# jzhou316/meta-gcn

Hardware: AMD Instinct MI355X
Metric: edges/sec GCN fwd+bwd, 10M-edge synth graph F=128, at 1/2/4/8 MI355X (higher is better)
Workload: dtype f32; 1 GPU; config2: Erdos-Renyi N=1M, E=10M (+1M self-loops), F=128, 3-layer GCN (sm, add, bias, ReLU) fwd+bwd; nodes=1000000, edges=10000000, nnz=11000000, feat=128, layers=3, global_batch=1, parallelism=single

## Files before the change

meta-gcn_amd/csrc/fused.hip:

```cpp

#include <string>

#include "mgcn_internal.h"
#include "x6.h"

#ifndef MGCN_NT_AUX
#define MGCN_NT_AUX 2
#endif
#ifndef MGCN_NT_OUT
#define MGCN_NT_OUT 2
#endif

namespace mgcn {
namespace {

using namespace x6;

constexpr int kXwF = 128;
constexpr int kXwRows = 32;
constexpr int kXwWaves = 8;
constexpr int kXwThreads = 64 * kXwWaves;
constexpr int kXwImg = kXwRows * 256;
constexpr int kXwStageLd = kXwF + 8;
constexpr int kXwStage = kXwRows * kXwStageLd * 4;
// ... 312 lines not shown
        wb[u] = bcast_g(mwb, grp, k & 31);
        const uint32_t oa = k < na ? (uint32_t)ca * ldx_b + 16u * gl : 0xfffffff0u;
        const uint32_t ob = k < nb ? (uint32_t)cb * ldx_b + 16u * gl : 0xfffffff0u;
        xa[u] = __builtin_bit_cast(float4, __builtin_amdgcn_raw_buffer_load_b128(rx, oa, 0, 0));
        xb[u] = __builtin_bit_cast(float4, __builtin_amdgcn_raw_buffer_load_b128(rx, ob, 0, 0));
        if constexpr (MAXM) {
          const int sa = bcast_g(msa, grp, k & 31);
          const int sb = bcast_g(msb, grp, k & 31);
          ba[u] = win[k < na ? (int64_t)sa * 4 + (gl >> 3) : 0];
          bb[u] = win[k < nb ? (int64_t)sb * 4 + (gl >> 3) : 0];
        }
      }
#pragma unroll
      for (int u = 0; u < U; ++u) {
        if constexpr (MAXM) {
          const uint32_t qa = ba[u] >> (4 * (gl & 7)), qb = bb[u] >> (4 * (gl & 7));
          xa[u].x = (qa & 1u) ? xa[u].x : 0.0f;
          xa[u].y = (qa & 2u) ? xa[u].y : 0.0f;
          xa[u].z = (qa & 4u) ? xa[u].z : 0.0f;
          xa[u].w = (qa & 8u) ? xa[u].w : 0.0f;
          xb[u].x = (qb & 1u) ? xb[u].x : 0.0f;
          xb[u].y = (qb & 2u) ? xb[u].y : 0.0f;
          xb[u].z = (qb & 4u) ? xb[u].z : 0.0f;
          xb[u].w = (qb & 8u) ? xb[u].w : 0.0f;
        }
        if (k0 + u < na) {
          aa[0] = __fadd_rn(aa[0], __fmul_rn(xa[u].x, wa[u]));
          aa[1] = __fadd_rn(aa[1], __fmul_rn(xa[u].y, wa[u]));
          aa[2] = __fadd_rn(aa[2], __fmul_rn(xa[u].z, wa[u]));
          aa[3] = __fadd_rn(aa[3], __fmul_rn(xa[u].w, wa[u]));
        }
        if (k0 + u < nb) {
          ab[0] = __fadd_rn(ab[0], __fmul_rn(xb[u].x, wb[u]));
          ab[1] = __fadd_rn(ab[1], __fmul_rn(xb[u].y, wb[u]));
          ab[2] = __fadd_rn(ab[2], __fmul_rn(xb[u].z, wb[u]));
          ab[3] = __fadd_rn(ab[3], __fmul_rn(xb[u].w, wb[u]));
        }
      }
    }
  }
}

struct RowSeq {
  int64_t base;
  int64_t step;
  int64_t n_rows;
  __device__ __forceinline__ int64_t row(int64_t k) const { return base + (k >> 1) * step + 16 * (k & 1); }
};

__device__ __forceinline__ int64_t my_chunks(int64_t n_chunks) {
  return blockIdx.x < n_chunks ? (n_chunks - 1 - blockIdx.x) / gridDim.x + 1 : 0;
}

__device__ __forceinline__ void store_row_terms(char *img_base, int lr, int gl, const float (&v)[4]) {
  uint32_t hi[2], mid[2], lo[2];
  split3_pair(f32x2{v[0], v[1]}, hi[0], mid[0], lo[0]);
  split3_pair(f32x2{v[2], v[3]}, hi[1], mid[1], lo[1]);
  char *img = img_base + img_off(lr, gl >> 1) + 8 * (gl & 1);
  *reinterpret_cast<uint2 *>(img) = make_uint2(hi[0], hi[1]);
  *reinterpret_cast<uint2 *>(img + kXwImg) = make_uint2(mid[0], mid[1]);
  *reinterpret_cast<uint2 *>(img + 2 * kXwImg) = make_uint2(lo[0], lo[1]);
}

__device__ __forceinline__ void mfma_rows(const char *img, const bf16x8 (&b)[3], int ks, int l16,
                                          int g4, f32x4_t (&acc)[2]) {
#pragma unroll
  for (int t = 0; t < 2; ++t) {
    const int off = img_off(16 * t + l16, 4 * ks + g4);
    const bf16x8 ah = *reinterpret_cast<const bf16x8 *>(img + off);
    const bf16x8 am = *reinterpret_cast<const bf16x8 *>(img + kXwImg + off);
    const bf16x8 al = *reinterpret_cast<const bf16x8 *>(img + 2 * kXwImg + off);
    acc[t] = mfma16_x6(ah, am, al, b[0], b[1], b[2], acc[t]);
  }
}

constexpr int kXfBuf = 3 * kXwImg;
constexpr int kXfStageOff = 2 * kXfBuf;
constexpr int kXfLds = kXfStageOff + 2 * kXfStage;
static_assert(2 * kXfLds <= 160 * 1024, "two forward workgroups per CU");

struct XwArgs {
  int64_t n_rows;
  const int64_t *rowptr;
  const int32_t *col;
  const float *w;
  const float *X;
  int64_t ldx;
  int64_t n_cols;
  const float *W;
  int64_t ldw;
  const float *bias;
  float *Y;
  int64_t ldy;
  uint32_t *relu_mask;
  float *Z;
  int64_t ldz;
  int mean;
  int relu;
  const uint32_t *pk;
  uint32_t pk_bytes, pk_rbits, pk_head;
  uint32_t pk_base[64];
};

template <int U, bool PK = false>
__global__ __launch_bounds__(kXwThreads, 2 * kXwPerCU) void spmm_xw_fwd_kernel(const XwArgs a) {
  __shared__ __attribute__((aligned(16))) char lds[kXfLds];
  const int tid = threadIdx.x;
  const int lane = tid & 63;
  const int wave = __builtin_amdgcn_readfirstlane(tid >> 6);
  const int gl = lane & 31, grp = lane >> 5;
  const int l16 = lane & 15, g4 = lane >> 4;
  const int64_t n_chunks = (a.n_rows + kXwRows - 1) / kXwRows;
  const bool has_b = a.bias != nullptr;
  const auto rx = buf_rsrc(PK ? nullptr : a.X, PK ? 0u : (uint32_t)(a.n_cols * a.ldx * 4));
  const uint32_t ldx_b = (uint32_t)a.ldx * 4u;
  Pk128 pk{};
  u32x2 hh[PK ? U : 1];
  if constexpr (PK) {
    pk.r = buf_rsrc(a.pk, a.pk_bytes);
    pk.rbits = a.pk_rbits;
    pk.head = a.pk_head;
    pk.base = a.pk_base[lane];
  }

  const int ncol = 16 * wave + l16;
  bf16x8 wb[4][3];
  {
    const float *wp = a.W + (int64_t)(8 * g4) * a.ldw + ncol;
#pragma unroll
    for (int ks = 0; ks < 4; ++ks) {
      float v[8];
#pragma unroll
      for (int j = 0; j < 8; ++j) v[j] = wp[(int64_t)(32 * ks + j) * a.ldw];
      split3_bf16(v, wb[ks][0], wb[ks][1], wb[ks][2]);
    }
  }
  const float bcol = has_b ? a.bias[ncol] : 0.0f;

  auto flush = [&](int64_t c, const float *stage) {
    const int64_t r0 = c * kXwRows;
    const int64_t left = a.n_rows - r0;
    const uint32_t rows_in = (uint32_t)(left >= kXwRows ? kXwRows : left);
    const auto ry = buf_rsrc(a.Y + r0 * a.ldy, rows_in * (uint32_t)a.ldy * 4u);
#pragma unroll
    for (int m = 0; m < 2; ++m) {
      const int lr = 16 * m + (tid >> 5);
      const float4 v = *reinterpret_cast<const float4 *>(stage + lr * kXwF + 4 * gl);
      __builtin_amdgcn_raw_buffer_store_b128(__builtin_bit_cast(u32x4, v), ry,
                                             4 * (int)(lr * a.ldy + 4 * gl), 0, MGCN_NT_OUT);
      if (a.relu_mask != nullptr) {
        const uint32_t m0 = (uint32_t)(__ballot(v.x > 0.0f) >> (32 * grp));
        const uint32_t m1 = (uint32_t)(__ballot(v.y > 0.0f) >> (32 * grp));
        const uint32_t m2 = (uint32_t)(__ballot(v.z > 0.0f) >> (32 * grp));
        const uint32_t m3 = (uint32_t)(__ballot(v.w > 0.0f) >> (32 * grp));
        if (gl == 0 && (uint32_t)lr < rows_in)
          *reinterpret_cast<uint4 *>(a.relu_mask + (r0 + lr) * 4) = make_uint4(m0, m1, m2, m3);
      }
    }
  };

  const int64_t n_my = my_chunks(n_chunks);
  const RowSeq seq{(int64_t)blockIdx.x * kXwRows + 2 * wave + grp, (int64_t)gridDim.x * kXwRows,
                   a.n_rows};
  RowMeta cur, nxt;
  meta_rowptr(a.rowptr, seq.row(0), seq.row(0) < a.n_rows, cur);
  if constexpr (PK) {
    meta_first_pk(pk, a.col, a.w, gl, cur);
    pk128_headers<U>(pk, cur.mc, grp, 0, cur.deg < 32 ? cur.deg : 32, 8u * (uint32_t)(gl >> 3), hh);
  } else {
    meta_first(a.col, a.w, gl, cur);
  }
  meta_rowptr(a.rowptr, seq.row(1), seq.row(1) < a.n_rows, nxt);
  int it = 0;
  for (int64_t chunk = blockIdx.x; chunk < n_chunks; chunk += gridDim.x, ++it) {
    char *buf = lds + (it & 1) * kXfBuf;
    float *stage = reinterpret_cast<float *>(lds + kXfStageOff + (it & 1) * kXfStage);

#pragma unroll 1
    for (int p = 0; p < 2; ++p) {
      const int lr = 16 * p + 2 * wave + grp;
      const int64_t k = 2 * it + p;
      if constexpr (PK)
        meta_first_pk(pk, a.col, a.w, gl, nxt);
      else
        meta_first(a.col, a.w, gl, nxt);
      RowMeta nn;
      const int64_t r2 = seq.row(k + 2);
      meta_rowptr(a.rowptr, r2, r2 < a.n_rows && k + 2 < 2 * n_my, nn);
      float acc[4];
      if constexpr (PK)
        gather_row_meta_pk<U>(pk, a.col, a.w, cur, nxt, gl, grp, acc, hh);
      else
        gather_row_meta<U>(rx, ldx_b, a.col, a.w, cur, gl, grp, acc);
      if (a.Z != nullptr) {
        const int64_t r0 = chunk * kXwRows;
        const int64_t left = a.n_rows - r0;
        const uint32_t rows_in = (uint32_t)(left >= kXwRows ? kXwRows : left);
        const auto rz = buf_rsrc(a.Z + r0 * a.ldz, rows_in * (uint32_t)a.ldz * 4u);
        __builtin_amdgcn_raw_buffer_store_b128(
            __builtin_bit_cast(u32x4, make_float4(acc[0], acc[1], acc[2], acc[3])), rz,
            4 * (int)(lr * a.ldz + 4 * gl), 0, MGCN_NT_AUX);
      }
      if (a.mean) {
        const float c = (float)(cur.deg > 1 ? cur.deg : 1);
#pragma unroll
        for (int j = 0; j < 4; ++j) acc[j] = __fdiv_rn(acc[j], c);
      }
      store_row_terms(buf, lr, gl, acc);
      cur = nxt;
      nxt = nn;
    }
    __syncthreads();
    if (it > 0)
      flush(chunk - gridDim.x, reinterpret_cast<const float *>(lds + kXfStageOff +
                                                                ((it + 1) & 1) * kXfStage));

    f32x4_t acc2[2];
#pragma unroll
    for (int t = 0; t < 2; ++t)
#pragma unroll
      for (int r = 0; r < 4; ++r) acc2[t][r] = 0.0f;
#pragma unroll
    for (int ks = 0; ks < 4; ++ks) mfma_rows(buf, wb[ks], ks, l16, g4, acc2);
#pragma unroll
    for (int t = 0; t < 2; ++t)
#pragma unroll
      for (int r = 0; r < 4; ++r) {
        float v = acc2[t][r];
        if (has_b) v = __fadd_rn(v, bcol);
        if (a.relu) v = (v < 0.0f) ? 0.0f : v;
        stage[(16 * t + 4 * g4 + r) * kXwF + ncol] = v;
      }
  }
  if (it > 0) {
    __syncthreads();
    flush(blockIdx.x + (int64_t)(it - 1) * gridDim.x,
          reinterpret_cast<const float *>(lds + kXfStageOff + ((it + 1) & 1) * kXfStage));
  }
}

constexpr int kXbHOff = 3 * kXwImg;
constexpr int kXbMaskOff = 6 * kXwImg;
constexpr int kXbDivOff = kXbMaskOff + kXwRows * 16;
constexpr int kXbStageOff = kXbDivOff + kXwRows * 4;
constexpr int kXbColsumOff = kXbStageOff + kXwStage;
constexpr int kXbLds = kXbColsumOff + kXwThreads * 16;
static_assert(2 * kXbLds <= 160 * 1024, "two backward workgroups per CU");

struct XbArgs {
  int64_t n_rows;
  const int64_t *rowptr;
  const int32_t *col;
  const float *w;
  const float *row_scale;
  const float *dY;
  int64_t lddy;
  int64_t n_cols;
  const float *X;
  int64_t ldx;
  const float *W;
  int64_t ldw;
  float *dX;
  int64_t lddx;
  const uint32_t *relu_mask;
  const float *row_div;
  float *dw_partial;
  float *colsum_partial;
  const uint32_t *win_mask;
  const int32_t *slot_map;
  const uint32_t *pk;
  uint32_t pk_bytes, pk_rbits, pk_head;
  uint32_t pk_base[64];
};

#ifdef MGCN_XW_PROFILE
__device__ unsigned long long g_xprof[2][64][6];
#define XPROF(it, k)                                                                      \
  if (blockIdx.x == 0 && (wave == 0 || wave == 7) && (it) < 64 && lane == 0)              \
    g_xprof[wave == 7][it][k] = __builtin_readcyclecounter();
#else
#define XPROF(it, k)
#endif

template <int U, bool DX, int EPI, bool MAXM, bool DW = true, bool PK = false>
__global__ __launch_bounds__(kXwThreads, 2 * kXwPerCU) void spmm_xw_bwd_kernel(const XbArgs a) {
  static_assert(!PK || (!DW && !MAXM), "the packed gather serves the dX-only adjoint");
  __shared__ __attribute__((aligned(16))) char lds[kXbLds];
  const int tid = threadIdx.x;
  const int lane = tid & 63;
  const int wave = __builtin_amdgcn_readfirstlane(tid >> 6);
  const int gl = lane & 31, grp = lane >> 5;
// ... 224 lines not shown
            stage[lc * kXwStageLd + kXwF + 4] = *reinterpret_cast<const float *>(lds + kXbDivOff + 4 * lc);
        }
      }
    }
    XPROF(it, 4);
    __syncthreads();
    XPROF(it, 5);
  }
  if constexpr (DX) {
    if (it > 0) flush(blockIdx.x + (int64_t)(it - 1) * gridDim.x);
  }

  float *slab = a.dw_partial + (int64_t)blockIdx.x * kXwF * kXwF;
#pragma unroll
  for (int s = 0; s < (DW ? 2 : 0); ++s)
#pragma unroll
    for (int r = 0; r < 16; ++r) {
      const int row = 32 * ti + (r & 3) + 8 * (r >> 2) + 4 * h;
      slab[row * kXwF + 32 * (tj0 + s) + lc] = accw[s][r];
    }
  if constexpr (DX && EPI != EPI_STORE) {
    __syncthreads();
    const float *red = reinterpret_cast<const float *>(lds + kXbColsumOff);
    if (tid < kXwF) {
      float c = 0.0f;
#pragma unroll
      for (int q = 0; q < 16; ++q) c = __fadd_rn(c, red[4 * (32 * q + (tid >> 2)) + (tid & 3)]);
      a.colsum_partial[(int64_t)blockIdx.x * kXwF + tid] = c;
    }
  }
}

int g_xw_unroll = 5;
int g_xw_pk_unroll = 3;
int g_xw_pk_bwd_unroll = 3;

int xw_grid() {
  int dev = 0, cus = 256;
  if (hipGetDevice(&dev) != hipSuccess ||
      hipDeviceGetAttribute(&cus, hipDeviceAttributeMultiprocessorCount, dev) != hipSuccess)
    cus = 256;
  return kXwPerCU * cus;
}

template <int U, bool PK = false>
int launch_xw(const XwArgs &a, hipStream_t s) {
  const int64_t n_chunks = (a.n_rows + kXwRows - 1) / kXwRows;
  int64_t grid = xw_grid();
  if (grid > n_chunks) grid = n_chunks;
  hipLaunchKernelGGL((spmm_xw_fwd_kernel<U, PK>), dim3((unsigned)grid), dim3(kXwThreads), 0, s, a);
  return check_launch("spmm_xw_fwd_kernel");
}

template <int U, bool DX, int EPI, bool MAXM, bool DW = true, bool PK = false>
int launch_xb(const XbArgs &a, int grid, hipStream_t s) {
  hipLaunchKernelGGL((spmm_xw_bwd_kernel<U, DX, EPI, MAXM, DW, PK>), dim3((unsigned)grid),
                     dim3(kXwThreads), 0, s, a);
  return check_launch("spmm_xw_bwd_kernel");
}

template <int U, bool PK = false>
int launch_xb_dx(const XbArgs &a, int epi, int grid, hipStream_t s) {
  if (epi == EPI_RELU_DIV) return launch_xb<U, true, EPI_RELU_DIV, false, false, PK>(a, grid, s);
  if (epi == EPI_RELU) return launch_xb<U, true, EPI_RELU, false, false, PK>(a, grid, s);
  return launch_xb<U, true, EPI_STORE, false, false, PK>(a, grid, s);
}

template <int U, bool MAXM>
int launch_xb_m(const XbArgs &a, int epi, int grid, hipStream_t s) {
  if (a.dX == nullptr) return launch_xb<U, false, EPI_STORE, MAXM>(a, grid, s);
  if (epi == EPI_RELU_DIV) return launch_xb<U, true, EPI_RELU_DIV, MAXM>(a, grid, s);
  if (epi == EPI_RELU) return launch_xb<U, true, EPI_RELU, MAXM>(a, grid, s);
  return launch_xb<U, true, EPI_STORE, MAXM>(a, grid, s);
}

template <int U>
int launch_xb_u(const XbArgs &a, int epi, int grid, hipStream_t s) {
  return a.win_mask != nullptr ? launch_xb_m<U, true>(a, epi, grid, s)
                               : launch_xb_m<U, false>(a, epi, grid, s);
}

constexpr int kBsDws = 2, kBsDwsH = 3, kBsDwsM = 4;
#ifndef MGCN_DS_MASK_RING
#define MGCN_DS_MASK_RING 1
#endif
constexpr int kBsImgSet = 3 * kXwImg;
constexpr int kDsXLd = kXwF + 4;
constexpr int kDsXOff = kBsImgSet;
constexpr int kDsMaskOff = kDsXOff + kXwRows * kDsXLd * 4;
constexpr int kDsDivOff = kDsMaskOff + kXwRows * 16;
constexpr int kDsRingBuf = kDsDivOff + kXwRows * 4;
constexpr int kDsWOff = 2 * kDsRingBuf;
constexpr int kDsCtrOff = kDsWOff + kXwF * kDsXLd * 4;
constexpr int kDsLds = kDsCtrOff + 64;
static_assert(kDsLds <= 160 * 1024, "one DWS workgroup per CU");
static_assert(16 * kXwF * 4 <= kDsWOff, "column-sum fold fits in the ring");
constexpr int kBsNG = 8, kBsNM = 8;
constexpr int kBsThreads = 64 * (kBsNG + kBsNM);

__device__ __forceinline__ int bs_lds_load(const int *p) {
  return __builtin_amdgcn_readfirstlane(
      __hip_atomic_load(p, __ATOMIC_RELAXED, __HIP_MEMORY_SCOPE_WORKGROUP));
}

__device__ __forceinline__ bool bs_wait_ge(const int *p, int target, int *abort_word,
                                           uint32_t limit) {
// ... 13 lines not shown
__device__ __forceinline__ int bs_signal(int *p, int v, int lane) {
  asm volatile("s_waitcnt lgkmcnt(0)" ::: "memory");
  int old = 0;
  if (lane == 0) old = __hip_atomic_fetch_add(p, v, __ATOMIC_RELAXED, __HIP_MEMORY_SCOPE_WORKGROUP);
  return __builtin_amdgcn_readfirstlane(old);
}

__device__ __forceinline__ f32x4_t mfma16_x6_at(const bf16x8 (&w)[3], const bf16x8 &xh,
                                               const bf16x8 &xm, const bf16x8 &xl, f32x4_t c) {
  c = __builtin_amdgcn_mfma_f32_16x16x32_bf16(w[0], xl, c, 0, 0, 0);
  c = __builtin_amdgcn_mfma_f32_16x16x32_bf16(w[2], xh, c, 0, 0, 0);
  c = __builtin_amdgcn_mfma_f32_16x16x32_bf16(w[1], xm, c, 0, 0, 0);
  c = __builtin_amdgcn_mfma_f32_16x16x32_bf16(w[0], xm, c, 0, 0, 0);
  c = __builtin_amdgcn_mfma_f32_16x16x32_bf16(w[1], xh, c, 0, 0, 0);
  return __builtin_amdgcn_mfma_f32_16x16x32_bf16(w[0], xh, c, 0, 0, 0);
}

struct XbsArgs {
  XbArgs b;
  float *hcs_partial;
  int dbg;
  uint32_t spin;
  unsigned *err;
};

template <int U, int EPI, int MODE>
__global__ __launch_bounds__(kBsThreads) void spmm_xw_bwd_ws_kernel(const XbsArgs A) {
  constexpr bool HCS = MODE == kBsDwsH;
  constexpr bool MAXM = MODE == kBsDwsM;
  constexpr bool MRING = MGCN_DS_MASK_RING;
  constexpr int kRing = kDsRingBuf;
  constexpr int kDbgMask = MAXM ? ~0 : mgcn::kDbgMask;
  const XbArgs &a = A.b;
  __shared__ __attribute__((aligned(16))) char lds[kDsLds];
  const int tid = threadIdx.x;
  const int lane = tid & 63;
  const int wave = __builtin_amdgcn_readfirstlane(tid >> 6);
  const int gl = lane & 31, grp = lane >> 5;
  const int l16 = lane & 15, g4 = lane >> 4;
  int *ctr = reinterpret_cast<int *>(lds + kDsCtrOff);
  int *filled = ctr, *mdone = ctr + 2, *freed = ctr + 4, *abort_word = ctr + 8;
  if (tid < 16) ctr[tid] = 0;
#pragma unroll
  for (int j = 0; j < 4; ++j) {
    const int e = tid + kBsThreads * j;
    const float4 v = *reinterpret_cast<const float4 *>(a.W + (int64_t)(e >> 5) * a.ldw + 4 * (e & 31));
    *reinterpret_cast<float4 *>(lds + kDsWOff + 4 * ((e >> 5) * kDsXLd + 4 * (e & 31))) = v;
  }
  __syncthreads();

  const int64_t n_chunks = (a.n_rows + kXwRows - 1) / kXwRows;
  const int64_t n_my = my_chunks(n_chunks);
  auto chunk_of = [&](int64_t i) { return (int64_t)blockIdx.x + i * gridDim.x; };
  auto rows_in = [&](int64_t c) -> uint32_t {
    const int64_t r = a.n_rows - c * kXwRows;
    return (uint32_t)(r <= 0 ? 0 : r >= kXwRows ? kXwRows : r);
  };

  float cs[4] = {0.0f, 0.0f, 0.0f, 0.0f};
  float hc[4] = {0.0f, 0.0f, 0.0f, 0.0f};
  f32x16 accw[2];
#pragma unroll
  for (int s = 0; s < 2; ++s)
#pragma unroll
    for (int r = 0; r < 16; ++r) accw[s][r] = 0.0f;

  if (wave < kBsNG) {
    const int64_t n_quads = 8 * n_my;
    auto row_of = [&](int64_t k, int second) -> int64_t {
      const int64_t q = wave + kBsNG * k;
      return chunk_of(q >> 3) * kXwRows + 4 * (q & 7) + 2 * second + grp;
    };
    const auto rdy = buf_rsrc(a.dY, (uint32_t)(a.n_cols * a.lddy * 4));
    const uint32_t ldy_b = (uint32_t)a.lddy * 4u;
    RowMeta cur[2] = {}, nxt[2] = {};
#pragma unroll
    for (int j = 0; j < 2; ++j) {
      meta_rowptr(a.rowptr, row_of(0, j), row_of(0, j) < a.n_rows && wave < n_quads, cur[j]);
      if constexpr (MAXM)
        meta_first_m(a.col, a.w, a.slot_map, gl, cur[j]);
      else
        meta_first(a.col, a.w, gl, cur[j]);
      meta_rowptr(a.rowptr, row_of(1, j), row_of(1, j) < a.n_rows && wave + kBsNG < n_quads,
                  nxt[j]);
    }
    int64_t k = 0;
    for (int64_t q = wave; q < n_quads; q += kBsNG, ++k) {
      RowMeta nn[2];
#pragma unroll
      for (int j = 0; j < 2; ++j) {
        if constexpr (MAXM)
          meta_first_m(a.col, a.w, a.slot_map, gl, nxt[j]);
        else
          meta_first(a.col, a.w, gl, nxt[j]);
        const int64_t r2 = row_of(k + 2, j);
        meta_rowptr(a.rowptr, r2, r2 < a.n_rows && q + 2 * kBsNG < n_quads, nn[j]);
      }
      const int64_t i = q >> 3;
      const int64_t c = chunk_of(i);
      const int64_t r0 = c * kXwRows;
      const int lr0 = 4 * (int)(q & 7) + grp;
      u32x4 zv[2] = {};
      if (!(A.dbg & kDbgMask & 4)) {
        const auto rz = buf_rsrc(a.X + r0 * a.ldx, rows_in(c) * (uint32_t)a.ldx * 4u);
#pragma unroll
        for (int j = 0; j < 2; ++j)
// ... 200 lines not shown
      }
      const int old = bs_signal(mdone + b, 1, lane);
      if (old == kBsNM * gen + kBsNM - 1) bs_signal(freed + b, 1, lane);
    }
  }
  __syncthreads();
  if (wave == 0 && bs_lds_load(abort_word) != 0) report_device_error(A.err, kDevErrDws);
  if (wave >= kBsNG) {
    const int m = wave - kBsNG;
    {
      const int h = lane >> 5, lc = lane & 31;
      const int ti = m >> 1, tj0 = 2 * (m & 1);
      float *slab = a.dw_partial + (int64_t)blockIdx.x * kXwF * kXwF;
#pragma unroll
      for (int s2 = 0; s2 < 2; ++s2)
#pragma unroll
        for (int r = 0; r < 16; ++r) {
          const int row = 32 * ti + (r & 3) + 8 * (r >> 2) + 4 * h;
          slab[row * kXwF + 32 * (tj0 + s2) + lc] = accw[s2][r];
        }
    }
    if constexpr (EPI != EPI_STORE) {
      float *red = reinterpret_cast<float *>(lds);
      *reinterpret_cast<float4 *>(red + l16 * kXwF + 16 * m + 4 * g4) =
          make_float4(cs[0], cs[1], cs[2], cs[3]);
    }
  }
  if constexpr (HCS) {
    float *red2 = reinterpret_cast<float *>(lds) + 16 * kXwF;
    if (wave < kBsNG)
      *reinterpret_cast<float4 *>(red2 + (2 * wave + grp) * kXwF + 4 * gl) =
          make_float4(hc[0], hc[1], hc[2], hc[3]);
  }
  if (EPI != EPI_STORE || HCS) {
    __syncthreads();
    if constexpr (EPI != EPI_STORE) {
      if (tid < kXwF) {
        const float *red = reinterpret_cast<const float *>(lds);
        float s = 0.0f;
#pragma unroll
        for (int l = 0; l < 16; ++l) s = __fadd_rn(s, red[l * kXwF + tid]);
        a.colsum_partial[(int64_t)blockIdx.x * kXwF + tid] = s;
      }
    }
    if (HCS && tid >= kXwF && tid < 2 * kXwF) {
      const int f = tid - kXwF;
      const float *red2 = reinterpret_cast<const float *>(lds) + 16 * kXwF;
      float s = 0.0f;
#pragma unroll
      for (int l = 0; l < 16; ++l) s = __fadd_rn(s, red2[l * kXwF + f]);
      A.hcs_partial[(int64_t)blockIdx.x * kXwF + f] = s;
    }
  }
}

int g_xw_ws_full = 1;
int g_xw_ws_max = 1;

int bs_grid() {
  int dev = 0, cus = 256;
  if (hipGetDevice(&dev) != hipSuccess ||
      hipDeviceGetAttribute(&cus, hipDeviceAttributeMultiprocessorCount, dev) != hipSuccess)
    cus = 256;
  return cus;
}

template <int U, int MODE>
int launch_bs_u(const XbsArgs &a, int epi, int grid, hipStream_t s) {
  if (epi == EPI_RELU_DIV)
    hipLaunchKernelGGL((spmm_xw_bwd_ws_kernel<U, EPI_RELU_DIV, MODE>), dim3(grid), dim3(kBsThreads),
                       0, s, a);
  else if (epi == EPI_RELU)
    hipLaunchKernelGGL((spmm_xw_bwd_ws_kernel<U, EPI_RELU, MODE>), dim3(grid), dim3(kBsThreads), 0,
                       s, a);
  else
    hipLaunchKernelGGL((spmm_xw_bwd_ws_kernel<U, EPI_STORE, MODE>), dim3(grid), dim3(kBsThreads), 0,
                       s, a);
  return check_launch("spmm_xw_bwd_ws_kernel");
}

int g_bs_dbg = 0;

int g_bs_full_unroll = 5;

template <int MODE>
int launch_bs(const XbsArgs &a, int epi, int grid, hipStream_t s) {
  if constexpr (MODE == kBsDwsM) {
    return launch_bs_u<3, MODE>(a, epi, grid, s);
  } else {
    return g_bs_full_unroll == 4 ? launch_bs_u<4, MODE>(a, epi, grid, s)
         : g_bs_full_unroll == 5 ? launch_bs_u<5, MODE>(a, epi, grid, s)
                                 : launch_bs_u<6, MODE>(a, epi, grid, s);
  }
}

int bs_prepare(XbsArgs &sa) {
  sa.dbg = MGCN_EXPERIMENT ? g_bs_dbg : 0;
  sa.spin = g_spin_limit;
  sa.err = device_error_word();
  return sa.err == nullptr ? MGCN_EHIP : MGCN_OK;
}

}

int xw_set_ws(const char *name, int value) {
  const std::string n(name);
  auto flag = [&](int &g) {
    if (value < 0 || value > 1) {
      set_error("%s must be 0 or 1", name);
      return (int)MGCN_EINVAL;
    }
    g = value;
    return (int)MGCN_OK;
  };
  auto unroll = [&](int &g, std::initializer_list<int> ok) {
    for (int v : ok)
      if (v == value) {
        g = value;
        return (int)MGCN_OK;
      }
    set_error("%s: unsupported value %d", name, value);
    return (int)MGCN_EINVAL;
  };
  if (n == "xw_pk_unroll" || n == "xw_pk_bwd_unroll") {
    if (!MGCN_EXPERIMENT) {
      set_error("%s: experiment builds only (make exp -> libmgcn_exp.so)", name);
      return MGCN_EINVAL;
    }
    return n == "xw_pk_unroll" ? unroll(g_xw_pk_unroll, {3, 4, 5, 6})
                               : unroll(g_xw_pk_bwd_unroll, {2, 3, 4});
  }
  if (n == "xw_ws_max") return flag(g_xw_ws_max);
  if (n == "xw_ws_full") return flag(g_xw_ws_full);
  if (n == "xw_ws_dbg") {
    if (!MGCN_EXPERIMENT) {
      set_error("xw_ws_dbg: experiment builds only (make exp -> libmgcn_exp.so)");
      return MGCN_EINVAL;
    }
    g_bs_dbg = value;
    return MGCN_OK;
  }
  return unroll(g_bs_full_unroll, {4, 5, 6});
}

int xw_set_unroll(int value) {
  if (value != 4 && value != 5 && value != 6 && value != 8) {
    set_error("spmm_xw_unroll must be 4, 5, 6 or 8 (5 / 6: the forward only)");
    return MGCN_EINVAL;
  }
  g_xw_unroll = value;
  return MGCN_OK;
}

}

using namespace mgcn;

extern "C" int mgcn_spmm_xw_supported(int32_t F_in, int32_t F_out, int reduce) {
  return F_in == F_out && (F_in == kXwF || F_in == 256) && gemm_precision_is_x6() &&
         (reduce == MGCN_REDUCE_SUM || reduce == MGCN_REDUCE_MEAN);
}

extern "C" int mgcn_spmm_xw_bwd_full_supported(int32_t F_in, int32_t F_out) {
  return F_in == kXwF && F_out == kXwF && gemm_precision_is_x6();
}

extern "C" size_t mgcn_spmm_xw_fwd_workspace_bytes(int32_t F_in, int32_t F_out) {
  return F_in == 256 && F_out == 256 ? xw_wide_workspace_bytes(false) : 0;
}

extern "C" int mgcn_spmm_xw_fwd(int64_t n_rows, int64_t n_cols, int32_t F_in, int32_t F_out,
                                const int64_t *rowptr, const int32_t *col, const float *w,
                                const float *X, int64_t ldx, const float *W, int64_t ldw,
                                const float *bias, float *Y, int64_t ldy, int reduce, int relu,
                                uint32_t *relu_mask, float *Z, int64_t ldz, void *workspace,
                                size_t workspace_bytes, void *stream) {
  clear_error();
  if (int rc = take_device_error()) return rc;
  MGCN_REQUIRE(n_rows >= 0, "mgcn_spmm_xw_fwd: negative size");
  MGCN_REQUIRE(mgcn_spmm_xw_supported(F_in, F_out, reduce),
               "mgcn_spmm_xw_fwd: unsupported F_in=%d F_out=%d reduce=%d (needs 128 x 128 or "
               "256 x 256, sum/mean, bf16x6)",
               F_in, F_out, reduce);
  MGCN_REQUIRE(relu_mask == nullptr || relu, "mgcn_spmm_xw_fwd: relu_mask needs relu");
  if (n_rows == 0) return MGCN_OK;
  MGCN_REQUIRE(rowptr && X && W && Y, "mgcn_spmm_xw_fwd: null array");
  MGCN_REQUIRE(ldx >= F_in && ldx % 4 == 0 && reinterpret_cast<uintptr_t>(X) % 16 == 0,
               "mgcn_spmm_xw_fwd: X must have 16-byte aligned rows");
  MGCN_REQUIRE(ldw >= F_out && ldy >= F_out, "mgcn_spmm_xw_fwd: leading dimension too small");
  if (F_in == 256) {
    MGCN_REQUIRE(n_cols > 0 && (uint64_t)16 * (uint64_t)(ldy > ldz ? ldy : ldz) * 4u < (1ull << 31),
                 "mgcn_spmm_xw_fwd: leading dimension too large");
    MGCN_REQUIRE(relu_mask == nullptr || reinterpret_cast<uintptr_t>(relu_mask) % 16 == 0,
                 "mgcn_spmm_xw_fwd: relu_mask not 16-byte aligned");
    MGCN_REQUIRE(Z == nullptr || (ldz >= F_in && ldz % 4 == 0 && reinterpret_cast<uintptr_t>(Z) % 16 == 0),
                 "mgcn_spmm_xw_fwd: Z must have 16-byte aligned rows (ldz >= F_in)");
    MGCN_REQUIRE(ldy % 4 == 0 && reinterpret_cast<uintptr_t>(Y) % 16 == 0,
                 "mgcn_spmm_xw_fwd: Y must have 16-byte aligned rows at F = 256");
    const size_t need = mgcn_spmm_xw_fwd_workspace_bytes(F_in, F_out);
    if (workspace == nullptr || workspace_bytes < need) {
      set_error("mgcn_spmm_xw_fwd: workspace %zu < %zu", workspace_bytes, need);
      return MGCN_EWORKSPACE;
    }
    return xw_wide_fwd(n_rows, rowptr, col, w, X, ldx, W, ldw, bias, Y, ldy,
                       reduce == MGCN_REDUCE_MEAN, relu != 0, relu_mask, Z, ldz, workspace,
                       as_stream(stream));
  }
  MGCN_REQUIRE(n_cols > 0 && (uint64_t)n_cols * (uint64_t)ldx * 4u <= 0xfffffff0ull,
               "mgcn_spmm_xw_fwd: X must hold 1 .. 4 GiB - 1 bytes (32-bit gather offsets)");
  MGCN_REQUIRE((uint64_t)kXwRows * (uint64_t)ldy * 4u < (1ull << 31),
               "mgcn_spmm_xw_fwd: ldy too large");
  MGCN_REQUIRE(bias == nullptr || reinterpret_cast<uintptr_t>(bias) % 4 == 0,
               "mgcn_spmm_xw_fwd: bias not 4-byte aligned");
  MGCN_REQUIRE(relu_mask == nullptr || reinterpret_cast<uintptr_t>(relu_mask) % 16 == 0,
               "mgcn_spmm_xw_fwd: relu_mask not 16-byte aligned");
  MGCN_REQUIRE(Z == nullptr || (ldz >= F_in && ldz % 4 == 0 && reinterpret_cast<uintptr_t>(Z) % 16 == 0 &&
                                (uint64_t)kXwRows * (uint64_t)ldz * 4u < (1ull << 31)),
               "mgcn_spmm_xw_fwd: Z must have 16-byte aligned rows (ldz >= F_in)");
  XwArgs a{};
  a.n_rows = n_rows;
  a.rowptr = rowptr;
  a.col = col;
  a.w = w;
  a.X = X;
  a.ldx = ldx;
  a.n_cols = n_cols;
  a.W = W;
  a.ldw = ldw;
  a.bias = bias;
  a.Y = Y;
  a.ldy = ldy;
  a.relu_mask = relu_mask;
  a.Z = Z;
  a.ldz = ldz;
  a.mean = reduce == MGCN_REDUCE_MEAN;
  a.relu = relu != 0;
  hipStream_t s = as_stream(stream);
  return g_xw_unroll == 4 ? launch_xw<4>(a, s)
       : g_xw_unroll == 5 ? launch_xw<5>(a, s)
       : g_xw_unroll == 6 ? launch_xw<6>(a, s)
                          : launch_xw<8>(a, s);
}

extern "C" size_t mgcn_spmm_xw_bwd_workspace_bytes(int64_t n_rows, int32_t F_in, int32_t F_out) {
  (void)n_rows;
  if (F_in == 256 && F_out == 256) return xw_wide_workspace_bytes(true);
  const size_t g = (size_t)xw_grid();
  return align_up(g * kXwF * kXwF * 4, 256) + align_up(g * kXwF * 4, 256);
}

namespace {
int xw_bwd_impl(int64_t n_rows, int64_t n_cols, int32_t F_in, int32_t F_out,
                const int64_t *rowptr_t, const int32_t *col_t, const float *w_t,
                const float *row_scale, const float *dY, int64_t lddy, const float *X,
                int64_t ldx, const float *W, int64_t ldw, float *dW, int64_t lddw, int accumulate,
                float *dX, int64_t lddx, const uint32_t *relu_mask, const float *row_div,
                float *colsum, const uint32_t *win_mask, const int32_t *slot_map,
                float *dy_colsum, void *workspace, size_t workspace_bytes, void *stream) {
  if (int rc = take_device_error()) return rc;
  MGCN_REQUIRE(n_rows >= 0, "mgcn_spmm_xw_bwd: negative size");
  MGCN_REQUIRE((win_mask == nullptr) == (slot_map == nullptr),
               "mgcn_spmm_xw_bwd: win_mask and slot_map go together (max adjoint)");
  MGCN_REQUIRE(mgcn_spmm_xw_supported(F_in, F_out, MGCN_REDUCE_SUM),
               "mgcn_spmm_xw_bwd: unsupported F_in=%d F_out=%d (needs 128 x 128 or 256 x 256, "
               "bf16x6)", F_in, F_out);
  const bool dx_only = X == nullptr && dW == nullptr;
  MGCN_REQUIRE(dx_only || mgcn_spmm_xw_bwd_full_supported(F_in, F_out),
               "mgcn_spmm_xw_bwd: at F=%d only the dX-only form (X = dW = NULL)", F_in);
  MGCN_REQUIRE(dx_only || (X != nullptr && dW != nullptr && lddw >= F_out),
               "mgcn_spmm_xw_bwd: bad dW (X and dW are given together, or both NULL for dX only)");
  MGCN_REQUIRE(row_div == nullptr || relu_mask != nullptr,
               "mgcn_spmm_xw_bwd: row_div needs relu_mask");
  hipStream_t s = as_stream(stream);
  if (n_rows == 0) {
    if (dy_colsum) MGCN_HIP_TRY(hipMemsetAsync(dy_colsum, 0, sizeof(float) * F_out, s));
    if (!accumulate && dW != nullptr)
      for (int32_t r = 0; r < F_in; ++r)
        MGCN_HIP_TRY(hipMemsetAsync(dW + r * lddw, 0, sizeof(float) * F_out, s));
    if (colsum && !(dx_only && accumulate))
      MGCN_HIP_TRY(hipMemsetAsync(colsum, 0, sizeof(float) * F_in, s));
    return MGCN_OK;
  }
  MGCN_REQUIRE(!dx_only || (dX != nullptr && win_mask == nullptr),
               "mgcn_spmm_xw_bwd: the dX-only form needs dX and takes no win_mask");
  const int epi = relu_mask == nullptr ? EPI_STORE : row_div != nullptr ? EPI_RELU_DIV : EPI_RELU;
  MGCN_REQUIRE(epi == EPI_STORE || (dX != nullptr && colsum != nullptr),
               "mgcn_spmm_xw_bwd: relu_mask needs dX and colsum");
  MGCN_REQUIRE(rowptr_t && dY, "mgcn_spmm_xw_bwd: null array");
  MGCN_REQUIRE(lddy >= F_out && lddy % 4 == 0 && reinterpret_cast<uintptr_t>(dY) % 16 == 0,
               "mgcn_spmm_xw_bwd: dY must have 16-byte aligned rows");
// ... 65 lines not shown
  float *hcs_partial = nullptr;
  if ((g_xw_ws_full || dy_colsum) && (win_mask == nullptr || (g_xw_ws_max && dX != nullptr))) {
    XbsArgs sa{};
    sa.b = a;
    if (int rc2 = bs_prepare(sa)) return rc2;
    grid = bs_grid() < n_chunks ? bs_grid() : (int)n_chunks;
    if (dy_colsum) hcs_partial = a.dw_partial + (size_t)grid * kXwF * kXwF;
    sa.hcs_partial = hcs_partial;
    rc = hcs_partial ? launch_bs<kBsDwsH>(sa, epi, grid, s)
         : win_mask  ? launch_bs<kBsDwsM>(sa, epi, grid, s)
                     : launch_bs<kBsDws>(sa, epi, grid, s);
  } else {
    rc = g_xw_unroll == 8 ? launch_xb_u<8>(a, epi, grid, s) : launch_xb_u<4>(a, epi, grid, s);
  }
  if (rc) return rc;
  rc = launch_split_reduce(a.dw_partial, grid, (int64_t)kXwF * kXwF, kXwF, dW, lddw, accumulate, s);
  if (rc == MGCN_OK && hcs_partial) rc = launch_colsum_fold(hcs_partial, grid, kXwF, dy_colsum, s);
  if (rc || epi == EPI_STORE) return rc;
  return launch_colsum_fold(a.colsum_partial, grid, kXwF, colsum, s);
}
}

extern "C" int mgcn_spmm_xw_bwd(int64_t n_rows, int64_t n_cols, int32_t F_in, int32_t F_out,
                                const int64_t *rowptr_t, const int32_t *col_t, const float *w_t,
                                const float *row_scale, const float *dY, int64_t lddy,
                                const float *X, int64_t ldx, const float *W, int64_t ldw,
                                float *dW, int64_t lddw, int accumulate, float *dX, int64_t lddx,
                                const uint32_t *relu_mask, const float *row_div, float *colsum,
                                const uint32_t *win_mask, const int32_t *slot_map,
                                void *workspace, size_t workspace_bytes, void *stream) {
  clear_error();
  return xw_bwd_impl(n_rows, n_cols, F_in, F_out, rowptr_t, col_t, w_t, row_scale, dY, lddy, X,
                     ldx, W, ldw, dW, lddw, accumulate, dX, lddx, relu_mask, row_div, colsum,
                     win_mask, slot_map, nullptr, workspace, workspace_bytes, stream);
}

extern "C" int mgcn_spmm_xw_bwd_hcs(int64_t n_rows, int64_t n_cols, const int64_t *rowptr_t,
                                    const int32_t *col_t, const float *w_t,
                                    const float *row_scale, const float *dY, int64_t lddy,
                                    const float *X, int64_t ldx, const float *W, int64_t ldw,
                                    float *dW, int64_t lddw, int accumulate, float *dX,
                                    int64_t lddx, const uint32_t *relu_mask,
                                    const float *row_div, float *colsum, float *dy_colsum,
                                    void *workspace, size_t workspace_bytes, void *stream) {
  clear_error();
  MGCN_REQUIRE(n_rows == n_cols, "mgcn_spmm_xw_bwd_hcs: needs n_rows == n_cols (%lld, %lld): "
               "every dY row a row of the view", (long long)n_rows, (long long)n_cols);
  MGCN_REQUIRE(X != nullptr && dW != nullptr && dX != nullptr && dy_colsum != nullptr,
               "mgcn_spmm_xw_bwd_hcs: X, dW, dX and dy_colsum are required");
  return xw_bwd_impl(n_rows, n_cols, kXwF, kXwF, rowptr_t, col_t, w_t, row_scale, dY, lddy, X,
                     ldx, W, ldw, dW, lddw, accumulate, dX, lddx, relu_mask, row_div, colsum,
                     nullptr, nullptr, dy_colsum, workspace, workspace_bytes, stream);
}

#ifdef MGCN_XW_PROFILE
extern "C" int mgcn_debug_xw_prof(unsigned long long *host) {
  MGCN_HIP_TRY(hipDeviceSynchronize());
  MGCN_HIP_TRY(hipMemcpyFromSymbol(host, HIP_SYMBOL(g_xprof), sizeof(g_xprof)));
  return MGCN_OK;
}
#endif

namespace {
int check_packed(const mgcn_packed_table *t, int32_t F, const char *who) {
  MGCN_REQUIRE(t != nullptr && t->words != nullptr, "%s: null packed table", who);
  MGCN_REQUIRE(t->F == F, "%s: packed table of F = %d for a layer of F = %d", who, t->F, F);
  MGCN_REQUIRE(t->n_seg >= 1 && t->n_seg <= 64, "%s: n_seg %d outside 1 .. 64", who, t->n_seg);
  MGCN_REQUIRE(t->row_bits >= 0 && t->row_bits + 6 <= 31 && t->seg_rows >= 1 &&
                   (int64_t)t->seg_rows <= ((int64_t)1 << t->row_bits),
               "%s: seg_rows %d does not fit row_bits %d", who, t->seg_rows, t->row_bits);
  MGCN_REQUIRE((uint64_t)t->seg_rows * (2 * (F / 32) + F) * 4u + 16u < (1ull << 31),
               "%s: seg_rows %d too large for the 2-GiB in-segment offsets", who, t->seg_rows);
  MGCN_REQUIRE(t->n_words >= 0, "%s: negative n_words", who);
  if (F == kXwF) {
    MGCN_REQUIRE((uint64_t)t->n_words * 4u <= 0x7ffffff0ull,
                 "%s: an F = 128 packed table spans at most 2 GiB - 16 B (got %lld words)", who,
                 (long long)t->n_words);
    for (int s = 0; s < t->n_seg; ++s)
      MGCN_REQUIRE(t->seg_base[s] >= 0 && t->seg_base[s] <= t->n_words,
                   "%s: segment %d at word %lld outside the table's %lld words", who, s,
                   (long long)t->seg_base[s], (long long)t->n_words);
  }
  return MGCN_OK;
}

template <class Args>
void fill_pk128(Args &a, const mgcn_packed_table *t) {
  a.pk = t->words;
  a.pk_bytes = (uint32_t)(t->n_words * 4);
  a.pk_rbits = (uint32_t)t->row_bits;
  a.pk_head = (uint32_t)t->seg_rows * 8u;
  for (int s = 0; s < 64; ++s) a.pk_base[s] = s < t->n_seg ? (uint32_t)t->seg_base[s] : 0u;
}
}

extern "C" int mgcn_spmm_xw_fwd_packed(int64_t n_rows, int32_t F_in, int32_t F_out,
                                       const int64_t *rowptr, const int32_t *col, const float *w,
                                       const mgcn_packed_table *X, const float *W, int64_t ldw,
                                       const float *bias, float *Y, int64_t ldy, int reduce,
                                       int relu, uint32_t *relu_mask, float *Z, int64_t ldz,
                                       void *workspace, size_t workspace_bytes, void *stream) {
  clear_error();
  if (int rc = take_device_error()) return rc;
  MGCN_REQUIRE(n_rows >= 0, "mgcn_spmm_xw_fwd_packed: negative size");
  MGCN_REQUIRE(mgcn_spmm_xw_supported(F_in, F_out, reduce),
               "mgcn_spmm_xw_fwd_packed: 128 x 128 or 256 x 256, sum / mean, bf16x6 only");
// ... 136 lines not shown
```

meta-gcn_amd/csrc/mgcn_internal.h:

```cpp
#pragma once

#include <hip/hip_runtime.h>

#include <atomic>
#include <cstdarg>
#include <cstdint>
#include <cstdio>

#include "mgcn.h"

namespace mgcn {

void set_error(const char *fmt, ...);
void clear_error();

inline hipStream_t as_stream(void *s) { return reinterpret_cast<hipStream_t>(s); }

#ifndef MGCN_EXPERIMENT
#define MGCN_EXPERIMENT 0
#endif
constexpr int kDbgMask = MGCN_EXPERIMENT ? ~0 : 0;
constexpr uint32_t kSpinLimitDefault = 1u << 25;
extern uint32_t g_spin_limit;

constexpr unsigned kDevErrDws = 1;
constexpr unsigned kDevErrWide = 2;
constexpr unsigned kDevErrPack = 3;
unsigned *device_error_word();
int take_device_error();

__device__ inline void report_device_error(unsigned *err, unsigned code) {
  if (err != nullptr && (threadIdx.x & 63) == 0)
    __hip_atomic_store(err, code, __ATOMIC_RELAXED, __HIP_MEMORY_SCOPE_SYSTEM);
}

inline int check_launch(const char *what) {
  hipError_t e = hipGetLastError();
  if (e != hipSuccess) {
    set_error("%s: %s", what, hipGetErrorString(e));
    return MGCN_EHIP;
  }
  return MGCN_OK;
}

#define MGCN_HIP_TRY(call)                                                    \
  do {                                                                        \
    hipError_t _e = (call);                                                   \
    if (_e != hipSuccess) {                                                   \
      ::mgcn::set_error("%s failed: %s (%s:%d)", #call, hipGetErrorString(_e), \
                        __FILE__, __LINE__);                                  \
      return MGCN_EHIP;                                                       \
    }                                                                         \
  } while (0)

#define MGCN_REQUIRE(cond, ...)       \
  do {                                \
    if (!(cond)) {                    \
      ::mgcn::set_error(__VA_ARGS__); \
      return MGCN_EINVAL;             \
    }                                 \
  } while (0)

inline size_t align_up(size_t x, size_t a) { return (x + a - 1) / a * a; }

inline unsigned grid_for(int64_t work_items, int block) {
  int64_t g = (work_items + block - 1) / block;
  if (g < 1) g = 1;
  if (g > 8192) g = 8192;
  return static_cast<unsigned>(g);
}

int gemm_set_tn_variant(int value);
int gemm_set_tn_staged(int value);
int gemm_set_precision(int value);
int gemm_precision_is_x6();
int xw_set_unroll(int value);
int xw_set_ws(const char *name, int value);
extern int g_fused_mask;
extern int g_rl_cap;
int launch_fold(const float *partial, int64_t splits, int64_t MN, int N, float *C, int64_t ldc,
                int accumulate, hipStream_t s);
int launch_fold_split(const float *partial, int64_t splits, int64_t MN, int N, float *C,
                      int64_t ldc, int N1, float *C2, int64_t ldc2, int accumulate, hipStream_t s);
int launch_split_reduce(const float *partial, int splits, int64_t MN, int N, float *C,
                        int64_t ldc, int accumulate, hipStream_t s);
int launch_colsum_fold(const float *partial, int64_t nparts, int N, float *out, hipStream_t s);
struct SideFold {
  const float *partial;
  int64_t parts, MN;
  int N, N1, log_eb, blocks;
  float *C, *C2;
  int64_t ldc, ldc2;
};
SideFold make_side_fold(const float *partial, int64_t parts, int64_t MN, int N, float *C,
                        int64_t ldc, int N1, float *C2, int64_t ldc2);
int launch_side_fold(const SideFold &f, hipStream_t s);

__device__ inline void side_fold_block(const SideFold &f, int b, float *red) {
  const int EB = 1 << f.log_eb, T = 256 >> f.log_eb;
  const int el = threadIdx.x & (EB - 1), g = threadIdx.x >> f.log_eb;
  const int64_t e = (int64_t)b * EB + el;
  float acc = 0.0f;
  if (e < f.MN) {
#pragma unroll 4
    for (int64_t sp = g; sp < f.parts; sp += T) acc = __fadd_rn(acc, f.partial[sp * f.MN + e]);
  }
  red[threadIdx.x] = acc;
  __syncthreads();
  for (int h = T >> 1; h >= 1; h >>= 1) {
    if (g < h) red[threadIdx.x] = __fadd_rn(red[threadIdx.x], red[threadIdx.x + h * EB]);
    __syncthreads();
  }
  if (g == 0 && e < f.MN) {
    const int64_t row = e / f.N, col = e % f.N;
    float *dst = col < f.N1 ? f.C + row * f.ldc + col : f.C2 + (col - f.N1) * f.ldc2 + row;
    *dst = red[el];
  }
}

struct TnJob {
  const float *A;
  int64_t lda;
  const float *B;
  int64_t ldb;
  int64_t K, kps;
  float *partial;
  int blocks;
};
bool tn_staged_plan(int64_t K, int32_t M, int32_t N, const float *A, int64_t lda, const float *B,
// ... 36 lines not shown
```

meta-gcn_amd/csrc/spmm.hip:

```cpp

#include <hipcub/hipcub.hpp>

#include "heavy.h"
#include "mgcn_internal.h"

namespace mgcn {
namespace {

constexpr int kWaves = 4;
constexpr int kBlock = 64 * kWaves;

template <int G>
__device__ __forceinline__ int bcast_i(int v, int group_base, int k) {
  if constexpr (G == 64) {
    return __builtin_amdgcn_readlane(v, k);
  } else {
    return __shfl(v, group_base + k, 64);
  }
}
template <int G>
__device__ __forceinline__ float bcast_f(float v, int group_base, int k) {
  return __int_as_float(bcast_i<G>(__float_as_int(v), group_base, k));
}

// ... 609 lines not shown
  clear_error();
  MGCN_REQUIRE(name != nullptr, "mgcn_set_option: null name");
  const std::string n(name);
  if (n == "spmm_vec") {
    MGCN_REQUIRE(value == 0 || value == 1 || value == 2 || value == 4, "spmm_vec must be 0,1,2,4");
    g_force_vec = value;
    return MGCN_OK;
  }
  if (n == "spmm_unroll") {
    MGCN_REQUIRE(value == 4 || value == 6 || value == 8 || value == 16,
                 "spmm_unroll must be 4, 6, 8 or 16");
    g_unroll = value;
    g_unroll_set = true;
    return MGCN_OK;
  }
  if (n == "heavy_lds_kb") {
    MGCN_REQUIRE(value >= 16 && value <= 160, "heavy_lds_kb must be in [16, 160]");
    g_heavy_lds = value * 1024;
    return MGCN_OK;
  }
  if (n == "heavy_block") {
    MGCN_REQUIRE(value == 256 || value == 512 || value == 1024, "heavy_block must be 256, 512 or 1024");
    g_heavy_block = value;
    return MGCN_OK;
  }
  if (n == "heavy_mid_q1") {
    MGCN_REQUIRE(value == 0 || value == 1, "heavy_mid_q1 must be 0 or 1");
    g_heavy_mid_q1 = value;
    return MGCN_OK;
  }
  if (n == "heavy_mid_lds_kb") {
    MGCN_REQUIRE(value >= 16 && value <= 160, "heavy_mid_lds_kb must be in [16, 160]");
    g_heavy_mid_lds = value * 1024;
    return MGCN_OK;
  }
  if (n == "heavy_giant_thr") {
    MGCN_REQUIRE(value >= 0, "heavy_giant_thr must be >= 0");
    g_giant_thr = value;
    return MGCN_OK;
  }
  if (n == "gemm_tn_variant") {
    MGCN_REQUIRE(value >= 0 && value <= 2, "gemm_tn_variant must be 0, 1 or 2");
    return gemm_set_tn_variant(value);
  }
  if (n == "gemm_tn_staged") {
    MGCN_REQUIRE(value == 0 || value == 1, "gemm_tn_staged must be 0 or 1");
    return gemm_set_tn_staged(value);
  }
  if (n == "gemm_precision") {
    MGCN_REQUIRE(value == 0 || value == 1, "gemm_precision must be 0 (f32) or 1 (bf16x6)");
    return gemm_set_precision(value);
  }
  if (n == "spmm_xw_unroll") return xw_set_unroll(value);
  if (n == "xw_ws_dbg" || n == "xw_ws_full" || n == "xw_ws_max" || n == "xw_ws_full_unroll" ||
      n == "xw_pk_unroll" || n == "xw_pk_bwd_unroll")
    return xw_set_ws(name, value);
  if (n == "wide_pair" || n == "wide_ws" || n == "wide_dbg" || n == "wide_mfma") return wide_set_option(name, value);
  if (n == "residual_blocks") {
    MGCN_REQUIRE(value >= 64 && value <= 65536, "residual_blocks must be in [64, 65536]");
    g_rl_cap = value;
    return MGCN_OK;
  }
  if (n == "residual_fused_mask") {
    MGCN_REQUIRE(value == 0 || value == 1, "residual_fused_mask must be 0 or 1");
    g_fused_mask = value;
    return MGCN_OK;
  }
  if (n == "heavy_side_fence") {
    MGCN_REQUIRE(value == 0 || value == 1, "heavy_side_fence must be 0 or 1");
    g_side_fence = value;
    return MGCN_OK;
  }
  if (n == "ws_spin_limit") {
    if (!MGCN_EXPERIMENT) {
      set_error("ws_spin_limit: experiment builds only (make exp -> libmgcn_exp.so)");
      return MGCN_EINVAL;
    }
    MGCN_REQUIRE(value >= 1, "ws_spin_limit must be >= 1");
    g_spin_limit = (uint32_t)value;
    return MGCN_OK;
  }
  if (n == "heavy_side_stream") {
    MGCN_REQUIRE(value == 0 || value == 1, "heavy_side_stream must be 0 or 1");
    g_heavy_side = value;
    return MGCN_OK;
  }
  set_error("mgcn_set_option: unknown option '%s'", name);
  return MGCN_EINVAL;
}

static int choose_vec(int32_t F, const void *p0, int64_t ld0, const void *p1, int64_t ld1) {
  int v = pick_vec(F, p0, ld0, p1, ld1);
  if (g_force_vec != 0 && g_force_vec < v) v = g_force_vec;
  return v;
}

extern "C" int mgcn_spmm_fwd(int64_t n_rows, int32_t F, const int64_t *rowptr, const int32_t *col,
                             const int32_t *eid, const float *w, const float *H, int64_t ldh,
                             float *Y, int64_t ldy, int reduce, const float *bias, int relu,
                             int32_t *argmax, uint32_t *win_mask, uint32_t *relu_mask,
                             const int32_t *order, int64_t n_heavy, int64_t n_giant,
                             void *stream) {
  clear_error();
  MGCN_REQUIRE(n_rows >= 0 && F >= 0, "mgcn_spmm_fwd: negative size");
  MGCN_REQUIRE(relu_mask == nullptr || (relu && F <= 128),
               "mgcn_spmm_fwd: relu_mask needs relu and F <= 128");
// ... 204 lines not shown
```

Before: 6.146 billion edges/s.

## Add dynamic tail chunk claiming to the fused SpMM-XW forward kernel

The dense forward fused SpMM+XW kernel gains a DYN mode. Every workgroup walks its static strided chunks up to dyn_first, and the last rounds are taken from a global atomic ticket counter, posted through a per-block mailbox two iterations ahead so the metadata prefetch pipeline keeps working. The goal is to even out the tail imbalance caused by varying row degrees. The cost is a hipMemsetAsync per launch, extra workspace, and atomic traffic. Timing probes guarded by MGCN_EXPERIMENT are also added.

```diff
diff --git a/meta-gcn_amd/csrc/fused.hip b/meta-gcn_amd/csrc/fused.hip
--- a/meta-gcn_amd/csrc/fused.hip
+++ b/meta-gcn_amd/csrc/fused.hip
@@ -388,6 +388,21 @@
   return blockIdx.x < n_chunks ? (n_chunks - 1 - blockIdx.x) / gridDim.x + 1 : 0;
 }
 
+#if MGCN_EXPERIMENT
+constexpr int kTailMaxWg = 1024;
+__device__ unsigned long long g_tail[2][kTailMaxWg][4];
+#define XTAIL_ENTRY(k)                                           \
+  if (threadIdx.x == 0 && blockIdx.x < kTailMaxWg) g_tail[k][blockIdx.x][0] = wall_clock64();
+#define XTAIL_EXIT(k, chunks)                                                         \
+  if ((threadIdx.x & 63) == 0 && blockIdx.x < kTailMaxWg) {                           \
+    atomicMax(&g_tail[k][blockIdx.x][1], (unsigned long long)wall_clock64());         \
+    if (threadIdx.x == 0) g_tail[k][blockIdx.x][2] = (unsigned long long)(chunks);    \
+  }
+#else
+#define XTAIL_ENTRY(k)
+#define XTAIL_EXIT(k, chunks)
+#endif
+
 __device__ __forceinline__ void store_row_terms(char *img_base, int lr, int gl, const float (&v)[4]) {
   uint32_t hi[2], mid[2], lo[2];
   split3_pair(f32x2{v[0], v[1]}, hi[0], mid[0], lo[0]);
@@ -433,13 +448,17 @@
   int64_t ldz;
   int mean;
   int relu;
+  int32_t dyn_first;
+  uint32_t *claim;
+  int32_t *mail;
   const uint32_t *pk;
   uint32_t pk_bytes, pk_rbits, pk_head;
   uint32_t pk_base[64];
 };
 
-template <int U, bool PK = false>
+template <int U, bool PK = false, bool DYN = false>
 __global__ __launch_bounds__(kXwThreads, 2 * kXwPerCU) void spmm_xw_fwd_kernel(const XwArgs a) {
+  static_assert(!(DYN && PK), "the dynamic claim serves the dense forward");
   __shared__ __attribute__((aligned(16))) char lds[kXfLds];
   const int tid = threadIdx.x;
   const int lane = tid & 63;
@@ -495,9 +514,15 @@
     }
   };
 
-  const int64_t n_my = my_chunks(n_chunks);
+  const int64_t n_my = my_chunks(DYN ? a.dyn_first : n_chunks);
   const RowSeq seq{(int64_t)blockIdx.x * kXwRows + 2 * wave + grp, (int64_t)gridDim.x * kXwRows,
                    a.n_rows};
+  XTAIL_ENTRY(0);
+  auto stat_chunk = [&](int i) -> int {
+    return i < (int)n_my ? (int)(blockIdx.x + i * gridDim.x) : -1;
+  };
+  int c1 = stat_chunk(1);
+  auto dyn_row = [&](int c, int p) { return (int64_t)c * kXwRows + 16 * p + 2 * wave + grp; };
   RowMeta cur, nxt;
   meta_rowptr(a.rowptr, seq.row(0), seq.row(0) < a.n_rows, cur);
   if constexpr (PK) {
@@ -508,7 +533,8 @@
   }
   meta_rowptr(a.rowptr, seq.row(1), seq.row(1) < a.n_rows, nxt);
   int it = 0;
-  for (int64_t chunk = blockIdx.x; chunk < n_chunks; chunk += gridDim.x, ++it) {
+  int prev = -1;
+  for (int64_t chunk = blockIdx.x; DYN ? chunk >= 0 : chunk < n_chunks; ++it) {
     char *buf = lds + (it & 1) * kXfBuf;
     float *stage = reinterpret_cast<float *>(lds + kXfStageOff + (it & 1) * kXfStage);
 
@@ -521,8 +547,8 @@
       else
         meta_first(a.col, a.w, gl, nxt);
       RowMeta nn;
-      const int64_t r2 = seq.row(k + 2);
-      meta_rowptr(a.rowptr, r2, r2 < a.n_rows && k + 2 < 2 * n_my, nn);
+      const int64_t r2 = DYN ? dyn_row(c1, p) : seq.row(k + 2);
+      meta_rowptr(a.rowptr, r2, r2 < a.n_rows && (DYN ? c1 >= 0 : k + 2 < 2 * n_my), nn);
       float acc[4];
       if constexpr (PK)
         gather_row_meta_pk<U>(pk, a.col, a.w, cur, nxt, gl, grp, acc, hh);
@@ -546,10 +572,21 @@
       cur = nxt;
       nxt = nn;
     }
+    uint32_t ticket = 0;
+    const bool draw = DYN && wave == 0 && it + 3 >= (int)n_my;
+    if constexpr (DYN)
+      if (draw && lane == 0)
+        ticket = __hip_atomic_fetch_add(a.claim, 1u, __ATOMIC_RELAXED, __HIP_MEMORY_SCOPE_AGENT);
     __syncthreads();
     if (it > 0)
-      flush(chunk - gridDim.x, reinterpret_cast<const float *>(lds + kXfStageOff +
-                                                                ((it + 1) & 1) * kXfStage));
+      flush(DYN ? prev : chunk - gridDim.x,
+            reinterpret_cast<const float *>(lds + kXfStageOff + ((it + 1) & 1) * kXfStage));
+    int posted = 0;
+    const bool take = DYN && it + 2 >= (int)n_my && it > 0;
+    if constexpr (DYN)
+      if (take)
+        posted = __hip_atomic_load(a.mail + 2 * blockIdx.x + ((it + 1) & 1), __ATOMIC_RELAXED,
+                                   __HIP_MEMORY_SCOPE_WORKGROUP);
 
     f32x4_t acc2[2];
 #pragma unroll
@@ -567,12 +604,28 @@
         if (a.relu) v = (v < 0.0f) ? 0.0f : v;
         stage[(16 * t + 4 * g4 + r) * kXwF + ncol] = v;
       }
+    if constexpr (DYN) {
+      if (draw && lane == 0)
+        __hip_atomic_store(a.mail + 2 * blockIdx.x + (it & 1), (int)ticket, __ATOMIC_RELAXED,
+                           __HIP_MEMORY_SCOPE_WORKGROUP);
+      int c2 = stat_chunk(it + 2);
+      if (take) {
+        const uint32_t c = (uint32_t)a.dyn_first + (uint32_t)__builtin_amdgcn_readfirstlane(posted);
+        c2 = c < (uint32_t)n_chunks ? (int)c : -1;
+      }
+      prev = (int)chunk;
+      chunk = c1;
+      c1 = c2;
+    } else {
+      chunk += gridDim.x;
+    }
   }
   if (it > 0) {
     __syncthreads();
-    flush(blockIdx.x + (int64_t)(it - 1) * gridDim.x,
+    flush(DYN ? prev : blockIdx.x + (int64_t)(it - 1) * gridDim.x,
           reinterpret_cast<const float *>(lds + kXfStageOff + ((it + 1) & 1) * kXfStage));
   }
+  XTAIL_EXIT(0, it);
 }
 
 constexpr int kXbHOff = 3 * kXwImg;
@@ -903,6 +956,32 @@
   return check_launch("spmm_xw_fwd_kernel");
 }
 
+int g_xw_dyn_rounds = 8;
+constexpr size_t kXwDynMailOff = 256;
+
+size_t xw_dyn_workspace_bytes() { return kXwDynMailOff + align_up((size_t)xw_grid() * 8, 256); }
+
+bool launch_xw_dyn(XwArgs &a, void *workspace, size_t workspace_bytes, hipStream_t s, int *rc) {
+  const int64_t n_chunks = (a.n_rows + kXwRows - 1) / kXwRows;
+  const int64_t grid = xw_grid();
+  const int64_t rounds = n_chunks / grid;
+  if (g_xw_dyn_rounds <= 0 || g_xw_unroll != 5 || workspace == nullptr ||
+      reinterpret_cast<uintptr_t>(workspace) % 4 != 0 || workspace_bytes < xw_dyn_workspace_bytes() || rounds < g_xw_dyn_rounds + 8 ||
+      n_chunks >= (int64_t(1) << 30))
+    return false;
+  a.dyn_first = (int32_t)((rounds - g_xw_dyn_rounds) * grid);
+  a.claim = static_cast<uint32_t *>(workspace);
+  a.mail = reinterpret_cast<int32_t *>(static_cast<char *>(workspace) + kXwDynMailOff);
+  if (hipMemsetAsync(a.claim, 0, sizeof(uint32_t), s) != hipSuccess) {
+    *rc = check_launch("hipMemsetAsync");
+    return true;
+  }
+  hipLaunchKernelGGL((spmm_xw_fwd_kernel<5, false, true>), dim3((unsigned)grid), dim3(kXwThreads),
+                     0, s, a);
+  *rc = check_launch("spmm_xw_fwd_kernel");
+  return true;
+}
+
 template <int U, bool DX, int EPI, bool MAXM, bool DW = true, bool PK = false>
 int launch_xb(const XbArgs &a, int grid, hipStream_t s) {
   hipLaunchKernelGGL((spmm_xw_bwd_kernel<U, DX, EPI, MAXM, DW, PK>), dim3((unsigned)grid),
@@ -1022,6 +1101,7 @@
   const int64_t n_chunks = (a.n_rows + kXwRows - 1) / kXwRows;
   const int64_t n_my = my_chunks(n_chunks);
   auto chunk_of = [&](int64_t i) { return (int64_t)blockIdx.x + i * gridDim.x; };
+  XTAIL_ENTRY(1);
   auto rows_in = [&](int64_t c) -> uint32_t {
     const int64_t r = a.n_rows - c * kXwRows;
     return (uint32_t)(r <= 0 ? 0 : r >= kXwRows ? kXwRows : r);
@@ -1328,6 +1408,7 @@
       A.hcs_partial[(int64_t)blockIdx.x * kXwF + f] = s;
     }
   }
+  XTAIL_EXIT(1, n_my);
 }
 
 int g_xw_ws_full = 1;
@@ -1419,6 +1500,15 @@
   return unroll(g_bs_full_unroll, {4, 5, 6});
 }
 
+int xw_set_dyn_rounds(int value) {
+  if (value < 0 || value > 64) {
+    set_error("xw_dyn_rounds must be in 0 .. 64 (0: no dynamic claim)");
+    return MGCN_EINVAL;
+  }
+  g_xw_dyn_rounds = value;
+  return MGCN_OK;
+}
+
 int xw_set_unroll(int value) {
   if (value != 4 && value != 5 && value != 6 && value != 8) {
     set_error("spmm_xw_unroll must be 4, 5, 6 or 8 (5 / 6: the forward only)");
@@ -1442,6 +1532,7 @@
 }
 
 extern "C" size_t mgcn_spmm_xw_fwd_workspace_bytes(int32_t F_in, int32_t F_out) {
+  if (F_in == kXwF && F_out == kXwF) return xw_dyn_workspace_bytes();
   return F_in == 256 && F_out == 256 ? xw_wide_workspace_bytes(false) : 0;
 }
 
@@ -1512,6 +1603,8 @@
   a.mean = reduce == MGCN_REDUCE_MEAN;
   a.relu = relu != 0;
   hipStream_t s = as_stream(stream);
+  int rc = MGCN_OK;
+  if (launch_xw_dyn(a, workspace, workspace_bytes, s, &rc)) return rc;
   return g_xw_unroll == 4 ? launch_xw<4>(a, s)
        : g_xw_unroll == 5 ? launch_xw<5>(a, s)
        : g_xw_unroll == 6 ? launch_xw<6>(a, s)
@@ -1683,6 +1776,17 @@
                      ldx, W, ldw, dW, lddw, accumulate, dX, lddx, relu_mask, row_div, colsum,
                      nullptr, nullptr, dy_colsum, workspace, workspace_bytes, stream);
 }
+
+#if MGCN_EXPERIMENT
+extern "C" int mgcn_debug_xw_tail(unsigned long long *host) {
+  MGCN_HIP_TRY(hipDeviceSynchronize());
+  if (host != nullptr)
+    MGCN_HIP_TRY(hipMemcpyFromSymbol(host, HIP_SYMBOL(g_tail), sizeof(g_tail)));
+  static const unsigned long long zero[2][kTailMaxWg][4] = {};
+  MGCN_HIP_TRY(hipMemcpyToSymbol(HIP_SYMBOL(g_tail), zero, sizeof(zero)));
+  return MGCN_OK;
+}
+#endif
 
 #ifdef MGCN_XW_PROFILE
 extern "C" int mgcn_debug_xw_prof(unsigned long long *host) {
diff --git a/meta-gcn_amd/csrc/mgcn_internal.h b/meta-gcn_amd/csrc/mgcn_internal.h
--- a/meta-gcn_amd/csrc/mgcn_internal.h
+++ b/meta-gcn_amd/csrc/mgcn_internal.h
@@ -75,6 +75,7 @@
 int gemm_set_precision(int value);
 int gemm_precision_is_x6();
 int xw_set_unroll(int value);
+int xw_set_dyn_rounds(int value);
 int xw_set_ws(const char *name, int value);
 extern int g_fused_mask;
 extern int g_rl_cap;
diff --git a/meta-gcn_amd/csrc/spmm.hip b/meta-gcn_amd/csrc/spmm.hip
--- a/meta-gcn_amd/csrc/spmm.hip
+++ b/meta-gcn_amd/csrc/spmm.hip
@@ -685,6 +685,7 @@
     return gemm_set_precision(value);
   }
   if (n == "spmm_xw_unroll") return xw_set_unroll(value);
+  if (n == "xw_dyn_rounds") return xw_set_dyn_rounds(value);
   if (n == "xw_ws_dbg" || n == "xw_ws_full" || n == "xw_ws_max" || n == "xw_ws_full_unroll" ||
       n == "xw_pk_unroll" || n == "xw_pk_bwd_unroll")
     return xw_set_ws(name, value);
```

After: 6.211 billion edges/s, median of 6. 1.1% higher.
